# widkyyu/Goal-conditioned-Reinforcement-Learning-with-environmental-and-policy-priors

Measured on AMD Instinct MI355X. Metric: env-steps/sec, higher is better.
Workload: dtype u8

## Files before the change

### goal-conditioned-reinforcement-learning-with-environmental-and-policy-priors_amd/_lib.py

```python
import ctypes as C
import os
import subprocess

_PKG_DIR = os.path.dirname(os.path.abspath(__file__))
LIB_PATH = os.path.join(_PKG_DIR, "libtwoarmy_hip.so")
CSRC_DIR = os.path.join(_PKG_DIR, "csrc")

TW_CELLS = 289
TW_REC_WORDS = 48
TW_DRAW_WORDS = 8
TW_F_AUTORESET = 1
TW_F_POLICY_IDX = 2
TW_F_MATRIX_CODE = 4
TW_F_SLAB_HIPMALLOC = 8

FIELDS = dict(AX=0, AY=1, DIR=2, STEP_COUNT=3, STEP_MOVE=4, PONE=5, PATROL=6, UP1=7, RIGHT2=8, UPD_LONG=9,
              UPD_HORIZ=10, RISK=11, FIRST_ROOM2=12, OBX=13, OBY=16, O1X=19, O1Y=22, O1_VALID=25, O2X=26,
              O2Y=30, O2_VALID=34, GOAL_X=35, GOAL_Y=36, T=37, ERROR=38, MAX_STEPS=39, EPISODES=40,
              LAST_REWARD=41, LAST_TERM=42, LAST_TRUNC=43, WALL_I1=44, WALL_I2=45)

ENV_ERRORS = {1: AttributeError, 2: AssertionError, 3: TypeError}


class TwoarmyLibraryError(RuntimeError):
    pass


def build(force=False):
    cmd = ["make", "-s", "-C", CSRC_DIR] + (["-B"] if force else [])
    subprocess.check_call(cmd)
    return LIB_PATH


_vp = C.c_void_p


class TwOutputs(C.Structure):
    _fields_ = [("obs", _vp), ("matrix", _vp), ("pos", _vp), ("reward", _vp), ("terminated", _vp), ("truncated", _vp),
                ("obs_pitch", C.c_int), ("mat_pitch", C.c_int), ("T", C.c_int), ("n_envs", C.c_int), ("flags", C.c_int),
                ("device", C.c_int), ("backing", C.c_int), ("slab_bytes", C.c_uint64), ("slab", _vp)]


_SIGS = {
    "tw_create": (C.c_int, [C.POINTER(_vp), C.c_int, C.c_int, C.c_int, C.c_int, C.c_uint64, C.c_uint32]),
    "tw_destroy": (C.c_int, [_vp]),
    "tw_reset": (C.c_int, [_vp, _vp, _vp, C.c_int, _vp]),
    "tw_step": (C.c_int, [_vp, _vp, _vp, _vp, C.c_int, _vp, C.c_int, _vp, _vp, _vp, _vp, C.c_int, _vp]),
    "tw_rollout": (C.c_int, [_vp, C.c_int, _vp, _vp, _vp, C.c_int, _vp, C.c_int, _vp, _vp, _vp, _vp, C.c_int, _vp]),
    "tw_set_envs_per_wave": (C.c_int, [_vp, C.c_int]),
    "tw_set_pipeline": (C.c_int, [_vp, C.c_int]),
    "tw_fallback_count": (C.c_int, [_vp, C.POINTER(C.c_int)]),
    "tw_fill_actions": (C.c_int, [_vp, C.c_int, _vp, _vp]),
    "tw_state_ptrs": (C.c_int, [_vp, C.POINTER(_vp), C.POINTER(_vp), C.POINTER(_vp)]),
    "tw_get_state_host": (C.c_int, [_vp, _vp, _vp, _vp]),
    "tw_set_state_host": (C.c_int, [_vp, _vp, _vp, _vp]),
    "tw_gen_obs": (C.c_int, [_vp, C.c_int, _vp, C.c_int, _vp]),
    "tw_n_envs": (C.c_int, [_vp]),
    "tw_view_size": (C.c_int, [_vp]),
    "tw_last_hip_error": (C.c_int, []),
    "tw_version": (C.c_char_p, []),
    "tw_build_id": (C.c_char_p, []),
    "tw_last_error_message": (C.c_char_p, []),
    "tw_alloc_outputs": (C.c_int, [_vp, C.c_int, C.c_int, C.POINTER(TwOutputs)]),
    "tw_free_outputs": (C.c_int, [C.POINTER(TwOutputs)]),
    "tw_abi_sizeof_outputs": (C.c_int, []),
    "tw_time_rollout": (C.c_int, [_vp, C.c_int, _vp, _vp, C.c_int, _vp, C.c_int, _vp, _vp, _vp, _vp, C.c_int, C.c_int, _vp,
                                  C.POINTER(C.c_float)]),
}

_f, _i, _u64, _i64 = C.c_float, C.c_int, C.c_uint64, C.c_int64
_SIGS.update({
    "ppo_sample": (C.c_int, [_vp, _i, _i, _vp, _u64, _u64, _vp, _vp, _vp]),
    "ppo_sample_dev": (C.c_int, [_vp, _i, _i, _vp, _u64, _u64, _vp, _vp, _vp, _vp]),
    "ppo_gae": (C.c_int, [_vp, _vp, _vp, _vp, _f, _f, _i, _i, _i, _vp, _vp, _vp, _vp]),
    "ppo_adv_norm": (C.c_int, [_vp, _i64, _f, _vp, _vp]),
    "ppo_loss_fwd_bwd": (C.c_int, [_vp, _vp, _vp, _vp, _vp, _vp, _i, _i, _f, _f, _vp, _vp, _vp, _vp, _vp]),
    "ppo_loss_fwd_bwd_masked": (C.c_int, [_vp, _vp, _vp, _vp, _vp, _vp, _i, _i, _i, _f, _f, _vp, _vp, _vp, _vp, _vp]),
    "ppo_gather_stack": (C.c_int, [_vp, _i, _vp, _i, _vp, _vp, _vp, _vp, _vp, _i, _vp, _vp, _vp]),
    "mg_gen_obs": (C.c_int, [_vp, _vp, _vp, _i, _i, _i, _vp, _vp, _vp, _vp, _i, _i, _vp, _i, _vp, _vp]),
    "mg_step": (C.c_int, [_vp, _vp, _i, _i, _i, _vp, _vp, _vp, _vp, _vp, _i, _vp, _vp, _vp, _vp, _vp]),
    "mg_render_tile_index": (C.c_int, [_i, _i, _i, _i, _i]),
    "mg_render_atlas_bytes": (_i64, [_i]),
    "mg_render_constants": (C.c_int, [C.POINTER(C.c_double)]),
    "mg_render_build_atlas": (C.c_int, [_i, _vp, _vp]),
    "mg_render": (C.c_int, [_vp, _vp, _vp, _i, _i, _i, _vp, _vp, _vp, _i, _vp, _i, _vp, _vp, _i, _vp, _i64, _vp, _vp]),
    "mg_highlight_mask": (C.c_int, [_vp, _i, _i, _i, _vp, _vp, _vp, _i, _i, _vp, _vp]),
    "ppo_her_relabel": (C.c_int, [_vp, _vp, _vp, _vp, _vp, _vp, _u64, C.c_uint32, C.c_uint32, _i, _i, _i, _vp, _vp, _vp,
                                  _vp, _vp, _vp, _vp, _vp]),
    "ppo_her_relabel_window": (C.c_int, [_vp, _vp, _vp, _vp, _vp, _vp, _u64, C.c_uint32, C.c_uint32, _i, _i, _i, _i, _vp,
                                         _vp, _vp, _vp, _vp, _vp, _vp, _vp]),
    "ppo_lstm_cell": (C.c_int, [_vp, _vp, C.c_longlong, _vp, _vp, _vp, _i, _i, _vp]),
    "ppo_decoder_frames": (C.c_int, [_vp, _i, _vp, _vp, _vp, _vp, _vp, C.c_float, _vp, _vp]),
    "ppo_gather_stack_u8": (C.c_int, [_vp, _i, _vp, _i, _vp, _vp, _vp, _vp, _vp, _i, _vp, _vp, _vp]),
    "ppo_age_scan": (C.c_int, [_vp, _vp, _vp, _i, _i, _vp, _vp]),
    "ppo_episode_scan": (C.c_int, [_vp, _vp, _vp, _i, _i, _vp, _vp, _vp, _vp, _vp]),
    "ppo_episode_summary": (C.c_int, [_vp, _vp, _vp, _vp, _vp, _vp, _i, _i, _i, C.c_double, C.c_double, _vp, _vp, _vp, _vp,
                                      _vp, _vp]),
    "ppo_episode_summary_workspace": (C.c_int, [_i, _i]),
    "ppo_bias_relu_nhwc": (C.c_int, [_vp, _vp, _i64, _i, _vp]),
    "ppo_conv1_up4_bias_relu": (C.c_int, [_vp, _i, _i, _vp, _vp, _vp, _vp]),
    "ppo_conv1_up4_bias_relu_c": (C.c_int, [_vp, _i, _i, _i, _vp, _vp, _vp, _vp]),
    "ppo_conv1_up4_bwd_groups": (C.c_int, [_i]),
    "ppo_conv1_up4_bwd": (C.c_int, [_vp, _i, _i, _vp, _vp, _vp, _vp, _vp]),
    "ppo_relu_bwd_bias_grad_nhwc_blocks": (C.c_int, [_i64, _i]),
    "ppo_relu_bwd_bias_grad_nhwc": (C.c_int, [_vp, _vp, _vp, _vp, _i64, _i, _vp]),
})

_lib = None


def exported_symbols():
    return sorted(_SIGS)


def lib():
    global _lib
    if _lib is None:
        if not os.path.exists(LIB_PATH):
            raise TwoarmyLibraryError(
                "%s not built: run `python -c 'import __graft_entry__ as g; g.build()'` "
                "(hipcc --offload-arch=gfx950); there is no CPU fallback" % LIB_PATH)
        import torch
        try:
            h = C.CDLL(LIB_PATH)
        except OSError as ex:
            raise TwoarmyLibraryError("cannot load %s: %s" % (LIB_PATH, ex)) from ex
        for name, (res, args) in _SIGS.items():
            try:
                fn = getattr(h, name)
            except AttributeError as ex:
                raise TwoarmyLibraryError("%s lacks symbol %s" % (LIB_PATH, name)) from ex
            fn.restype, fn.argtypes = res, args
        runtimes = set()
        try:
            with open("/proc/self/maps") as f:
                for line in f:
                    if "libamdhip64" in line:
                        runtimes.add(line.split()[-1])
        except OSError:
            pass
        if h.tw_abi_sizeof_outputs() != C.sizeof(TwOutputs):
            raise TwoarmyLibraryError("struct tw_outputs: the library has %d bytes, the ctypes mirror %d"
                                      % (h.tw_abi_sizeof_outputs(), C.sizeof(TwOutputs)))
        if len(runtimes) > 1:
            raise TwoarmyLibraryError("two HIP runtimes mapped (%s): import torch before loading %s"
                                      % (sorted(runtimes), LIB_PATH))
        _lib = h
    return _lib


def check(rc, what):
    if rc != 0:
        raise TwoarmyLibraryError("%s failed: rc=%d hipError=%d %s" % (
            what, rc, lib().tw_last_hip_error(), lib().tw_last_error_message().decode()))
```

### goal-conditioned-reinforcement-learning-with-environmental-and-policy-priors_amd/csrc/ppo_kernels.hip

```cpp

#include <hip/hip_runtime.h>
#include <float.h>
#include <stdint.h>

#include "twoarmy.h"
#include "twoarmy_ppo.h"

namespace {

constexpr float CAT_EPS = FLT_EPSILON;

__device__ __forceinline__ void philox4x32_10(uint32_t k0, uint32_t k1, uint32_t &c0, uint32_t &c1, uint32_t &c2,
                                              uint32_t &c3) {
#pragma unroll
    for (int r = 0; r < 10; ++r) {
        const uint32_t lo0 = 0xD2511F53u * c0, hi0 = __umulhi(0xD2511F53u, c0);
        const uint32_t lo1 = 0xCD9E8D57u * c2, hi1 = __umulhi(0xCD9E8D57u, c2);
        const uint32_t n0 = hi1 ^ c1 ^ k0, n2 = hi0 ^ c3 ^ k1;
        c0 = n0; c1 = lo1; c2 = n2; c3 = lo0;
        k0 += 0x9E3779B9u; k1 += 0xBB67AE85u;
    }
}

template <int A>
__global__ void ppo_sample_kernel(const float *__restrict__ probs, int B, const float *__restrict__ uniforms,
                                  uint32_t k0, uint32_t k1, uint64_t offset, const uint64_t *__restrict__ offset_dev,
                                  int32_t *__restrict__ action, float *__restrict__ logp) {
    const int b = blockIdx.x * blockDim.x + threadIdx.x;
    if (b >= B) return;
    float p[A];
    float sum = 0.f;
#pragma unroll
    for (int k = 0; k < A; ++k) { p[k] = probs[(size_t)b * A + k]; sum += p[k]; }
    float u;
    if (uniforms) u = uniforms[b];
    else {
        const uint64_t ctr = (uint64_t)b + offset + (offset_dev ? *offset_dev : 0ull);
        uint32_t c0 = (uint32_t)ctr, c1 = (uint32_t)(ctr >> 32), c2 = 0, c3 = 0x54574F53u;
        philox4x32_10(k0, k1, c0, c1, c2, c3);
        u = (float)(c0 >> 8) * (1.0f / 16777216.0f);
    }
    int a = A - 1, last = A - 1;
    float cum = 0.f, qa = 0.f;
    bool found = false;
#pragma unroll
    for (int k = 0; k < A; ++k) {
        const float q = p[k] / sum;
        cum += q;
        if (q > 0.f) last = k;
        if (!found && cum > u) { a = k; found = true; }
    }
    if (!found) a = last;
#pragma unroll
    for (int k = 0; k < A; ++k) if (k == a) qa = p[k] / sum;
    action[b] = a;
    logp[b] = logf(fminf(fmaxf(qa, CAT_EPS), 1.0f - CAT_EPS));
}

__global__ __launch_bounds__(256) void ppo_bias_relu_kernel(float4 *__restrict__ y, const float4 *__restrict__ bias,
                                                            size_t n4, int c4) {
    const size_t stride = (size_t)gridDim.x * blockDim.x;
    for (size_t i = (size_t)blockIdx.x * blockDim.x + threadIdx.x; i < n4; i += stride) {
        float4 v = y[i];
        const float4 b = bias[i % c4];
        v.x = fmaxf(v.x + b.x, 0.f); v.y = fmaxf(v.y + b.y, 0.f);
        v.z = fmaxf(v.z + b.z, 0.f); v.w = fmaxf(v.w + b.w, 0.f);
        y[i] = v;
    }
}

__global__ __launch_bounds__(256) void ppo_relu_bwd_bias_grad_kernel(const float4 *__restrict__ gy,
                                                                     const float4 *__restrict__ y,
                                                                     float4 *__restrict__ gx,
                                                                     float4 *__restrict__ partial, size_t n_pixels,
                                                                     int c4, int pixels_per_block) {
    __shared__ float4 red[256];
    const int rows = 256 / c4;
    const int cq = threadIdx.x % c4, row = threadIdx.x / c4;
    const size_t p0 = (size_t)blockIdx.x * pixels_per_block;
    const size_t p1 = p0 + pixels_per_block < n_pixels ? p0 + pixels_per_block : n_pixels;
    float4 acc = make_float4(0.f, 0.f, 0.f, 0.f);
    if (row < rows) {
        for (size_t px = p0 + row; px < p1; px += rows) {
            const size_t i = px * c4 + cq;
            const float4 g = gy[i], v = y[i];
            float4 o;
            o.x = v.x > 0.f ? g.x : 0.f; o.y = v.y > 0.f ? g.y : 0.f;
            o.z = v.z > 0.f ? g.z : 0.f; o.w = v.w > 0.f ? g.w : 0.f;
            gx[i] = o;
            acc.x += o.x; acc.y += o.y; acc.z += o.z; acc.w += o.w;
        }
    }
    red[threadIdx.x] = acc;
    __syncthreads();
    if (row == 0) {
        for (int r = 1; r < rows; ++r) {
            const float4 o = red[r * c4 + cq];
            acc.x += o.x; acc.y += o.y; acc.z += o.z; acc.w += o.w;
        }
        partial[(size_t)blockIdx.x * c4 + cq] = acc;
    }
}

template <int F, int CQ>
__global__ __launch_bounds__(256) void ppo_conv1_up4_kernel(const float *__restrict__ frames, const float4 *__restrict__ wf,
                                                            const float4 *__restrict__ bias, float4 *__restrict__ out, int B) {
    __shared__ float xs[F * 18 * 18];
    constexpr int SLOTS = 256 / CQ;
    const int b = blockIdx.x, tid = threadIdx.x;
    const int cq = tid % CQ, slot = tid / CQ;
    const float *src = frames + (size_t)b * F * 289;
    for (int i = tid; i < F * 324; i += 256) {
        const int c = i / 324, r = i - c * 324, y = r / 18, x = r - y * 18;
        xs[i] = (y < 17 && x < 17) ? src[c * 289 + y * 17 + x] : 0.f;
    }
    __syncthreads();
    const float4 bv = bias[cq];
    float4 *dst = out + (size_t)b * 1089 * CQ;
#pragma unroll 1
    for (int ph = 0; ph < 4; ++ph) {
        const int py = ph >> 1, px = ph & 1;
        float4 w[4 * F];
#pragma unroll
        for (int k = 0; k < 4 * F; ++k) w[k] = wf[(ph * 4 * F + k) * CQ + cq];
        const int ny = 17 - py, nx = 17 - px;
        for (int q = slot; q < ny * nx; q += SLOTS) {
            const int m = q / nx, n = q - m * nx;
            float4 acc = bv;
#pragma unroll
            for (int t = 0; t < 4; ++t) {
                const int ty = t >> 1, tx = t & 1;
#pragma unroll
                for (int c = 0; c < F; ++c) {
                    const float xv = xs[c * 324 + (m + ty) * 18 + n + tx];
                    const float4 ww = w[t * F + c];
                    acc.x = fmaf(xv, ww.x, acc.x); acc.y = fmaf(xv, ww.y, acc.y);
                    acc.z = fmaf(xv, ww.z, acc.z); acc.w = fmaf(xv, ww.w, acc.w);
                }
            }
            acc.x = fmaxf(acc.x, 0.f); acc.y = fmaxf(acc.y, 0.f); acc.z = fmaxf(acc.z, 0.f); acc.w = fmaxf(acc.w, 0.f);
            dst[((2 * m + py) * 33 + 2 * n + px) * CQ + cq] = acc;
        }
    }
}

template <int F>
__global__ __launch_bounds__(256) void ppo_conv1_up4_bwd_kernel(const float *__restrict__ frames, const float4 *__restrict__ gy,
                                                                const float4 *__restrict__ y, float4 *__restrict__ gw_part,
                                                                float4 *__restrict__ gb_part, int B) {
    __shared__ float xs[F * 18 * 18];
    __shared__ float4 red[256];
    const int tid = threadIdx.x, cq = tid & 15, slot = tid >> 4;
    const int ph = blockIdx.y, py = ph >> 1, px = ph & 1;
    const int ny = 17 - py, nx = 17 - px;
    float4 acc[4 * F];
#pragma unroll
    for (int k = 0; k < 4 * F; ++k) acc[k] = make_float4(0.f, 0.f, 0.f, 0.f);
    float4 accb = make_float4(0.f, 0.f, 0.f, 0.f);
    for (int b = blockIdx.x; b < B; b += gridDim.x) {
        __syncthreads();
        const float *src = frames + (size_t)b * F * 289;
        for (int i = tid; i < F * 324; i += 256) {
            const int c = i / 324, r = i - c * 324, yy = r / 18, xx = r - yy * 18;
            xs[i] = (yy < 17 && xx < 17) ? src[c * 289 + yy * 17 + xx] : 0.f;
        }
        __syncthreads();
        const size_t base = (size_t)b * 1089 * 16;
        for (int q = slot; q < ny * nx; q += 16) {
            const int m = q / nx, n = q - m * nx;
            const size_t o = base + (size_t)((2 * m + py) * 33 + 2 * n + px) * 16 + cq;
            const float4 gv = gy[o], yv = y[o];
            float4 g;
            g.x = yv.x > 0.f ? gv.x : 0.f; g.y = yv.y > 0.f ? gv.y : 0.f;
            g.z = yv.z > 0.f ? gv.z : 0.f; g.w = yv.w > 0.f ? gv.w : 0.f;
            accb.x += g.x; accb.y += g.y; accb.z += g.z; accb.w += g.w;
#pragma unroll
            for (int t = 0; t < 4; ++t) {
                const int ty = t >> 1, tx = t & 1;
#pragma unroll
                for (int c = 0; c < F; ++c) {
                    const float xv = xs[c * 324 + (m + ty) * 18 + n + tx];
                    float4 &a = acc[t * F + c];
                    a.x = fmaf(xv, g.x, a.x); a.y = fmaf(xv, g.y, a.y); a.z = fmaf(xv, g.z, a.z); a.w = fmaf(xv, g.w, a.w);
                }
            }
        }
    }
    const size_t wbase = ((size_t)blockIdx.x * 4 + ph) * (4 * F) * 16;
#pragma unroll
    for (int k = 0; k <= 4 * F; ++k) {
        __syncthreads();
        red[tid] = k < 4 * F ? acc[k < 4 * F ? k : 0] : accb;
        __syncthreads();
        if (slot == 0) {
            float4 sum = red[cq];
            for (int r = 1; r < 16; ++r) {
                const float4 o = red[r * 16 + cq];
                sum.x += o.x; sum.y += o.y; sum.z += o.z; sum.w += o.w;
            }
            if (k < 4 * F) gw_part[wbase + (size_t)k * 16 + cq] = sum;
            else gb_part[((size_t)blockIdx.x * 4 + ph) * 16 + cq] = sum;
        }
    }
}

constexpr int GT = 64;

template <int GN>
__global__ __launch_bounds__(256) void ppo_gae_kernel(const float *__restrict__ reward, const float *__restrict__ value,
                                                      const float *__restrict__ next_value,
                                                      const uint8_t *__restrict__ done, float gamma, float lambda,
                                                      int use_done_mask, int T, int N, float *__restrict__ adv,
                                                      float *__restrict__ target, float *__restrict__ ret) {
    __shared__ float sd[GT][GN + 1];
    __shared__ float sc[GT][GN + 1];
    __shared__ float carry[GN];
    constexpr int ROWS = 256 / GN;
    const int tid = threadIdx.x, tx = tid % GN, ty = tid / GN;
    const int n = blockIdx.x * GN + tx;
    if (tid < GN) carry[tid] = 0.f;
    const int nchunks = (T + GT - 1) / GT;
    for (int ch = nchunks - 1; ch >= 0; --ch) {
        const int t0 = ch * GT;
        __syncthreads();
        for (int r = ty; r < GT; r += ROWS) {
            const int t = t0 + r;
            float d = 0.f, c = 1.f;
            if (t < T && n < N) {
                const size_t i = (size_t)t * N + n;
                const float cut = (use_done_mask && done[i]) ? 0.f : 1.f;
                const float tv = reward[i] + (gamma * next_value[i]) * cut;
                if (target) target[i] = tv;
                d = tv - value[i];
                c = gamma * lambda * cut;
            }
            sd[r][tx] = d; sc[r][tx] = c;
        }
        __syncthreads();
        const int wave = tid >> 6, lane = tid & 63;
        for (int e = wave * (GN / 4); e < (wave + 1) * (GN / 4); ++e) {
            float d = sd[lane][e], c = sc[lane][e];
#pragma unroll
            for (int off = 1; off < 64; off <<= 1) {
                const float d2 = __shfl_down(d, off), c2 = __shfl_down(c, off);
                if (lane + off < 64 && c != 0.f) { d = fmaf(c, d2, d); c = c * c2; }
            }
            const float a = c != 0.f ? fmaf(c, carry[e], d) : d;
            sd[lane][e] = a;
            const float a0 = __shfl(a, 0);
            if (lane == 0) carry[e] = a0;
        }
        __syncthreads();
        for (int r = ty; r < GT; r += ROWS) {
            const int t = t0 + r;
            if (t < T && n < N) {
                const size_t i = (size_t)t * N + n;
                const float a = sd[r][tx];
                if (adv) adv[i] = a;
                if (ret) ret[i] = a + value[i];
            }
        }
    }
}

__global__ __launch_bounds__(256) void ppo_moments_kernel(const float *__restrict__ x, int64_t n, double *__restrict__ ws) {
    __shared__ double s1[256], s2[256];
    double a = 0.0, b = 0.0;
    for (int64_t i = (int64_t)blockIdx.x * 256 + threadIdx.x; i < n; i += (int64_t)gridDim.x * 256) {
        const double v = (double)x[i];
        a += v; b += v * v;
    }
    s1[threadIdx.x] = a; s2[threadIdx.x] = b;
    __syncthreads();
    for (int s = 128; s > 0; s >>= 1) {
        if ((int)threadIdx.x < s) { s1[threadIdx.x] += s1[threadIdx.x + s]; s2[threadIdx.x] += s2[threadIdx.x + s]; }
        __syncthreads();
    }
    if (threadIdx.x == 0) { ws[2 * blockIdx.x] = s1[0]; ws[2 * blockIdx.x + 1] = s2[0]; }
}

__global__ __launch_bounds__(256) void ppo_normalise_kernel(float *__restrict__ x, int64_t n, float eps,
                                                            const double *__restrict__ ws, int nblocks) {
    __shared__ float s_mean, s_inv;
    __shared__ double r1[256], r2[256];
    r1[threadIdx.x] = (int)threadIdx.x < nblocks ? ws[2 * threadIdx.x] : 0.0;
// ... 722 lines not shown
    const int64_t per_block = (M + nblocks - 1) / nblocks;
    const int per_thread = (int)((per_block + 255) / 256);
    hipStream_t st = (hipStream_t)stream;
    hipLaunchKernelGGL(ppo_episode_partial_kernel, dim3(nblocks), dim3(256), 0, st, ep_return, ep_length, terminated,
                       truncated, reward, action, M, per_block, per_thread, keep, gain, workspace);
    hipLaunchKernelGGL(ppo_episode_finalize_kernel, dim3(1), dim3(64), 0, st, workspace, nblocks, A, score, summary,
                       action_hist, reward_hist);
    return check_launch();
}

int ppo_bias_relu_nhwc(float *y, const float *bias, int64_t n_pixels, int C, void *stream) {
    if (!y || !bias || n_pixels <= 0 || C <= 0 || (C & 3) || ((uintptr_t)y & 15u) || ((uintptr_t)bias & 15u)) return TW_E_ARG;
    const size_t n4 = (size_t)n_pixels * (C / 4);
    const int grid = (int)((n4 + 255) / 256 < 8192 ? (n4 + 255) / 256 : 8192);
    hipLaunchKernelGGL(ppo_bias_relu_kernel, dim3(grid), dim3(256), 0, (hipStream_t)stream, reinterpret_cast<float4 *>(y),
                       reinterpret_cast<const float4 *>(bias), n4, C / 4);
    return check_launch();
}

int ppo_relu_bwd_bias_grad_nhwc_blocks(int64_t n_pixels, int C) {
    if (n_pixels <= 0 || C <= 0 || (C & 3) || C > 256) return TW_E_ARG;
    const int64_t want = (n_pixels + 511) / 512;
    return (int)(want < 4096 ? want : 4096);
}

int ppo_relu_bwd_bias_grad_nhwc(const float *gy, const float *y, float *gx, float *partial, int64_t n_pixels, int C,
                                void *stream) {
    const int blocks = ppo_relu_bwd_bias_grad_nhwc_blocks(n_pixels, C);
    if (blocks <= 0 || !gy || !y || !gx || !partial || (((uintptr_t)gy | (uintptr_t)y | (uintptr_t)gx | (uintptr_t)partial) & 15u))
        return TW_E_ARG;
    const int ppb = (int)((n_pixels + blocks - 1) / blocks);
    hipLaunchKernelGGL(ppo_relu_bwd_bias_grad_kernel, dim3(blocks), dim3(256), 0, (hipStream_t)stream,
                       reinterpret_cast<const float4 *>(gy), reinterpret_cast<const float4 *>(y),
                       reinterpret_cast<float4 *>(gx), reinterpret_cast<float4 *>(partial), (size_t)n_pixels, C / 4, ppb);
    return check_launch();
}

int ppo_conv1_up4_bias_relu(const float *frames, int B, int F, const float *folded_w, const float *bias, float *out,
                            void *stream) {
    return ppo_conv1_up4_bias_relu_c(frames, B, F, 64, folded_w, bias, out, stream);
}

int ppo_conv1_up4_bias_relu_c(const float *frames, int B, int F, int C_out, const float *folded_w, const float *bias,
                              float *out, void *stream) {
    if (!frames || !folded_w || !bias || !out || B <= 0 || ((uintptr_t)out & 15u) || ((uintptr_t)folded_w & 15u) ||
        ((uintptr_t)bias & 15u))
        return TW_E_ARG;
    hipStream_t st = (hipStream_t)stream;
#define PPO_CONV1_LAUNCH(FF, CQQ)                                                                                        \
    hipLaunchKernelGGL((ppo_conv1_up4_kernel<FF, CQQ>), dim3(B), dim3(256), 0, st, frames,                               \
                       reinterpret_cast<const float4 *>(folded_w), reinterpret_cast<const float4 *>(bias),               \
                       reinterpret_cast<float4 *>(out), B)
    if (F == 4 && C_out == 64) PPO_CONV1_LAUNCH(4, 16);
    else if (F == 8 && C_out == 64) PPO_CONV1_LAUNCH(8, 16);
    else if (F == 1 && C_out == 16) PPO_CONV1_LAUNCH(1, 4);
    else return TW_E_ARG;
#undef PPO_CONV1_LAUNCH
    return check_launch();
}

int ppo_conv1_up4_bwd_groups(int B) { return B <= 0 ? TW_E_ARG : (B < 256 ? B : 256); }

int ppo_conv1_up4_bwd(const float *frames, int B, int F, const float *gy, const float *y, float *gw_partial,
                      float *gb_partial, void *stream) {
    const int groups = ppo_conv1_up4_bwd_groups(B);
    if (groups <= 0 || !frames || !gy || !y || !gw_partial || !gb_partial ||
        (((uintptr_t)gy | (uintptr_t)y | (uintptr_t)gw_partial | (uintptr_t)gb_partial) & 15u))
        return TW_E_ARG;
    hipStream_t st = (hipStream_t)stream;
    const dim3 grid(groups, 4), block(256);
    if (F == 4)
        hipLaunchKernelGGL(ppo_conv1_up4_bwd_kernel<4>, grid, block, 0, st, frames, reinterpret_cast<const float4 *>(gy),
                           reinterpret_cast<const float4 *>(y), reinterpret_cast<float4 *>(gw_partial),
                           reinterpret_cast<float4 *>(gb_partial), B);
    else if (F == 8)
        hipLaunchKernelGGL(ppo_conv1_up4_bwd_kernel<8>, grid, block, 0, st, frames, reinterpret_cast<const float4 *>(gy),
                           reinterpret_cast<const float4 *>(y), reinterpret_cast<float4 *>(gw_partial),
                           reinterpret_cast<float4 *>(gb_partial), B);
    else
        return TW_E_ARG;
    return check_launch();
}

int ppo_decoder_frames(const float *z, int n_frames, const float *w1, const float *b1, const float *w2, const float *b2,
                       const float *kfold, float b3, float *frames, void *stream) {
    if (!z || !w1 || !b1 || !w2 || !b2 || !kfold || !frames || n_frames <= 0) return TW_E_ARG;
    const int grid = n_frames < 512 ? n_frames : 512;
    hipLaunchKernelGGL(ppo_decoder_frames_kernel, dim3(grid), dim3(256), 0, (hipStream_t)stream, z, n_frames, w1, b1, w2,
                       b2, kfold, b3, frames);
    return check_launch();
}

int ppo_lstm_cell(const float *gates_a, const float *gates_b, long long ldb, const float *bias, float *c, float *h, int B,
                  int H, void *stream) {
    if ((!gates_a && !gates_b) || !c || !h || B <= 0 || H <= 0 || (H & 3) ||
        (((uintptr_t)gates_a | (uintptr_t)c | (uintptr_t)h) & 15u))
        return TW_E_ARG;
    if (gates_b && ((((uintptr_t)gates_b) & 15u) || (ldb & 3) || ldb < 4LL * H)) return TW_E_ARG;
    if (bias && (((uintptr_t)bias) & 15u)) return TW_E_ARG;
    const long long n = (long long)B * (H / 4);
    if (n > 0x7fffffffLL) return TW_E_ARG;
    hipLaunchKernelGGL(ppo_lstm_cell_kernel, dim3((unsigned)((n + 255) / 256)), dim3(256), 0, (hipStream_t)stream,
                       reinterpret_cast<const float4 *>(gates_a), reinterpret_cast<const float4 *>(gates_b), ldb / 4,
                       reinterpret_cast<const float4 *>(bias), reinterpret_cast<float4 *>(c), reinterpret_cast<float4 *>(h),
                       B, H / 4);
    return check_launch();
}

}
```

### goal-conditioned-reinforcement-learning-with-environmental-and-policy-priors_amd/ppo_ops.py

```python
import ctypes as C

import torch

from . import _lib


def _p(t, dtype=None):
    if t is None:
        return None
    assert t.is_cuda and t.is_contiguous(), "PPO kernels take contiguous device tensors"
    if dtype is not None:
        assert t.dtype == dtype, "expected %s got %s" % (dtype, t.dtype)
    return C.c_void_p(t.data_ptr())


def _stream(t):
    return C.c_void_p(torch.cuda.current_stream(t.device).cuda_stream)


def sample(probs, uniforms=None, seed=0, offset=0, offset_dev=None):
    B, A = probs.shape
    action = torch.empty(B, dtype=torch.int32, device=probs.device)
    logp = torch.empty(B, dtype=torch.float32, device=probs.device)
    _lib.check(_lib.lib().ppo_sample_dev(_p(probs, torch.float32), B, A, _p(uniforms, torch.float32), seed, offset,
# ... 130 lines not shown
    _lib.check(fn(*args, None, _p(counts), None, None, None, None, None, _stream(pos)), "ppo_her_relabel_window")
    incl = torch.cumsum(counts.long(), 0)
    H = int(incl[-1])
    offsets = (incl - counts.long()).contiguous()
    out = dict(t=torch.empty(H, dtype=torch.int32, device=dev), n=torch.empty(H, dtype=torch.int32, device=dev),
               goal=torch.empty((H, 2), dtype=torch.float32, device=dev),
               reward=torch.empty(H, dtype=torch.float32, device=dev), done=torch.empty(H, dtype=torch.uint8, device=dev),
               counts=counts)
    if H:
        _lib.check(fn(*args, _p(offsets), _p(counts), _p(out["t"]), _p(out["n"]), _p(out["goal"]), _p(out["reward"]),
                      _p(out["done"]), _stream(pos)), "ppo_her_relabel_window")
    return out


class _ConvBiasReLU(torch.autograd.Function):

    @staticmethod
    def forward(ctx, x, w, b, stride):
        y = torch.ops.aten.convolution(x, w, None, list(stride), [0, 0], [1, 1], False, [0, 0], 1)
        assert y.is_contiguous(memory_format=torch.channels_last), "conv epilogue kernels need channels-last activations"
        B, Cc, H, W = y.shape
        _lib.check(_lib.lib().ppo_bias_relu_nhwc(C.c_void_p(y.data_ptr()), _p(b.detach(), torch.float32), B * H * W, Cc,
                                                 _stream(y)), "ppo_bias_relu_nhwc")
        ctx.save_for_backward(x, w, y)
        ctx.stride = list(stride)
        return y

    @staticmethod
    def backward(ctx, gy):
        x, w, y = ctx.saved_tensors
        gy = gy.contiguous(memory_format=torch.channels_last)
        B, Cc, H, W = y.shape
        npix = B * H * W
        blocks = _lib.lib().ppo_relu_bwd_bias_grad_nhwc_blocks(npix, Cc)
        g = torch.empty_like(y)
        partial = torch.empty((blocks, Cc), dtype=torch.float32, device=y.device)
        _lib.check(_lib.lib().ppo_relu_bwd_bias_grad_nhwc(C.c_void_p(gy.data_ptr()), C.c_void_p(y.data_ptr()),
                                                          C.c_void_p(g.data_ptr()), _p(partial), npix, Cc, _stream(y)),
                   "ppo_relu_bwd_bias_grad_nhwc")
        gx, gw, _ = torch.ops.aten.convolution_backward(g, x, w, None, ctx.stride, [0, 0], [1, 1], False, [0, 0], 1,
                                                        [bool(ctx.needs_input_grad[0]), True, False])
        return gx, gw, partial.sum(0), None


def conv_bias_relu(x, weight, bias, stride):
    assert x.is_cuda and x.dtype == torch.float32 and x.is_contiguous(memory_format=torch.channels_last)
    return _ConvBiasReLU.apply(x, weight, bias, tuple(stride))


def fold_conv1_weights(w):
    O, F = w.shape[0], w.shape[1]
    w = w.detach().reshape(O, F, 4, 4).float()
    z = torch.zeros_like(w[:, :, 0:1, :])
    rows = torch.stack([torch.cat([w.sum(2, keepdim=True), z], 2),
                        torch.cat([w[:, :, 0:2].sum(2, keepdim=True), w[:, :, 2:4].sum(2, keepdim=True)], 2)], 0)
    zc = torch.zeros_like(rows[..., 0:1])
    cols = torch.stack([torch.cat([rows.sum(-1, keepdim=True), zc], -1),
                        torch.cat([rows[..., 0:2].sum(-1, keepdim=True), rows[..., 2:4].sum(-1, keepdim=True)], -1)], 1)
    return cols.permute(0, 1, 4, 5, 3, 2).contiguous()


@torch.no_grad()
def conv1_up4_bias_relu_infer(frames, weight, bias):
    B, F, _ = frames.shape
    Cout = weight.shape[0]
    y = torch.empty((B, Cout, 33, 33), dtype=torch.float32, device=frames.device, memory_format=torch.channels_last)
    wf = fold_conv1_weights(weight)
    _lib.check(_lib.lib().ppo_conv1_up4_bias_relu_c(_p(frames.contiguous(), torch.float32), B, F, Cout, _p(wf),
                                                    _p(bias.contiguous(), torch.float32), C.c_void_p(y.data_ptr()),
                                                    _stream(y)), "ppo_conv1_up4_bias_relu_c")
    return y


class _Conv1Up4(torch.autograd.Function):

    @staticmethod
    def forward(ctx, frames, w, b, wf):
        B, F, _ = frames.shape
        y = torch.empty((B, w.shape[0], 33, 33), dtype=torch.float32, device=frames.device,
                        memory_format=torch.channels_last)
        if wf is None:
            wf = fold_conv1_weights(w)
        fr = frames.contiguous()
        _lib.check(_lib.lib().ppo_conv1_up4_bias_relu(_p(fr, torch.float32), B, F, _p(wf), _p(b.detach().contiguous()),
                                                      C.c_void_p(y.data_ptr()), _stream(y)), "ppo_conv1_up4_bias_relu")
        ctx.save_for_backward(fr, w, y)
        return y

    @staticmethod
    def backward(ctx, gy):
        fr, w, y = ctx.saved_tensors
        gy = gy.contiguous(memory_format=torch.channels_last)
        B, F = fr.shape[0], fr.shape[1]
        groups = _lib.lib().ppo_conv1_up4_bwd_groups(B)
        gw_part = torch.empty((groups, 2, 2, 2, 2, F, 64), dtype=torch.float32, device=y.device)
        gb_part = torch.empty((groups, 4, 64), dtype=torch.float32, device=y.device)
        _lib.check(_lib.lib().ppo_conv1_up4_bwd(_p(fr, torch.float32), B, F, C.c_void_p(gy.data_ptr()), C.c_void_p(y.data_ptr()),
                                                _p(gw_part), _p(gb_part), _stream(y)), "ppo_conv1_up4_bwd")
        return None, unfold_conv1_grad(gw_part.sum(0)).to(w.dtype), gb_part.sum((0, 1)), None


def unfold_conv1_grad(gwf):
    ty = torch.tensor([[0, 0, 0, 0], [0, 0, 1, 1]], device=gwf.device)
    out = None
    for py in (0, 1):
        for px in (0, 1):
            g = gwf[py, px][ty[py]][:, ty[px]]
            out = g if out is None else out + g
    return out.permute(3, 2, 0, 1).contiguous()


def conv1_up4_bias_relu(frames, weight, bias, folded=None):
    assert frames.is_cuda and frames.dtype == torch.float32 and weight.shape[2:] == (4, 4) and weight.shape[0] == 64
    return _Conv1Up4.apply(frames, weight, bias, folded)


def fold_decoder_tail(w3):
    m = torch.tensor([[0., 0., 1., 1.], [1., 1., 1., 1.], [1., 1., 0., 0.]], dtype=w3.dtype, device=w3.device)
    return torch.einsum("ur,crs,vs->cuv", m, w3[:, 0], m).mul_(1.0 / 16.0).contiguous()


def decoder_frames(z, w1, b1, w2, b2, w3, b3):
    assert z.dim() == 4 and tuple(z.shape[1:]) == (64, 4, 4) and z.dtype == torch.float32
    z = z.contiguous()
    n = z.shape[0]
    out = torch.empty((n, 289), dtype=torch.float32, device=z.device)
    if n:
        _lib.check(_lib.lib().ppo_decoder_frames(_p(z), n, _p(w1.detach().contiguous(), torch.float32),
                                                 _p(b1.detach().contiguous(), torch.float32),
                                                 _p(w2.detach().contiguous(), torch.float32),
                                                 _p(b2.detach().contiguous(), torch.float32),
                                                 _p(fold_decoder_tail(w3.detach())), 0.0, _p(out), _stream(z)),
                   "ppo_decoder_frames")
        out += b3.detach().view(1, 1)
    return out


def lstm_cell_(gates, c, gates_b=None, bias=None):
    B, H = c.shape
    H4 = 4 * H
    assert c.dtype == torch.float32 and (gates is not None or gates_b is not None)
    assert gates is None or (gates.shape == (B, H4) and gates.dtype == torch.float32)
    pb, ldb = None, 0
    if gates_b is not None:
        assert gates_b.shape == (B, H4) and gates_b.stride(1) == 1 and gates_b.dtype == torch.float32 and gates_b.is_cuda
        pb, ldb = C.c_void_p(gates_b.data_ptr()), gates_b.stride(0) if B > 1 else H4
    h = torch.empty_like(c)
    _lib.check(_lib.lib().ppo_lstm_cell(_p(gates), pb, ldb, _p(bias), _p(c), _p(h), B, H, _stream(c)), "ppo_lstm_cell")
    return h
```

### include/twoarmy_ppo.h

```cpp
#ifndef TWOARMY_PPO_H
#define TWOARMY_PPO_H

#include <stdint.h>

#ifdef __cplusplus
extern "C" {
#endif

int ppo_sample(const float *probs, int B, int A, const float *uniforms, uint64_t seed, uint64_t offset,
               int32_t *action, float *logp, void *stream);
int ppo_sample_dev(const float *probs, int B, int A, const float *uniforms, uint64_t seed, uint64_t offset,
                   const uint64_t *offset_dev, int32_t *action, float *logp, void *stream);

int ppo_gae(const float *reward, const float *value, const float *next_value, const uint8_t *done,
            float gamma, float lambda, int use_done_mask, int T, int N, float *adv, float *target, float *ret,
            void *stream);

int ppo_adv_norm(float *adv, int64_t n, float eps, double *workspace, void *stream);

int ppo_loss_fwd_bwd(const float *probs, const int32_t *action, const float *old_logp, const float *adv,
                     const float *value, const float *target_v, int B, int A, float clip, float ent_coef,
                     float *losses, float *grad_probs, float *grad_value, float *workspace, void *stream);
int ppo_loss_fwd_bwd_masked(const float *probs, const int32_t *action, const float *old_logp, const float *adv,
                            const float *value, const float *target_v, int B, int n_valid, int A, float clip,
                            float ent_coef, float *losses, float *grad_probs, float *grad_value, float *workspace,
                            void *stream);

int ppo_gather_stack(const float *frames, int frame_pitch, const float *pos_frames, int N,
                     const int32_t *k_idx, const int32_t *n_idx, const int32_t *age, const float *init_frame,
                     const float *init_pos, int B, float *out, float *pos_out, void *stream);

int ppo_gather_stack_u8(const uint8_t *frames, int frame_pitch, const float *pos_frames, int N,
                        const int32_t *k_idx, const int32_t *n_idx, const int32_t *age, const float *init_frame,
                        const float *init_pos, int B, float *out, float *pos_out, void *stream);

int ppo_age_scan(const uint8_t *terminated, const uint8_t *truncated, const int32_t *age0, int T, int N,
                 int32_t *age, void *stream);

int ppo_episode_scan(const float *reward, const uint8_t *terminated, const uint8_t *truncated, int T, int N,
                     double *carry_return, int32_t *carry_length, double *ep_return, int32_t *ep_length, void *stream);

int ppo_episode_summary(const double *ep_return, const int32_t *ep_length, const uint8_t *terminated,
                        const uint8_t *truncated, const float *reward, const int32_t *action, int A, int T, int N,
                        double keep, double gain, double *score, double *summary, int64_t *action_hist,
                        int64_t *reward_hist, double *workspace, void *stream);
int ppo_episode_summary_workspace(int T, int N);

int ppo_her_relabel(const float *pos, const uint8_t *terminated, const uint8_t *truncated, const int32_t *age0,
                    const float *reward, const int32_t *choices, uint64_t seed, uint32_t env_id0, uint32_t step0, int T,
                    int N, int max_goals, const int64_t *offsets, int32_t *counts, int32_t *out_t, int32_t *out_n,
                    float *out_goal, float *out_reward, uint8_t *out_done, void *stream);
int ppo_her_relabel_window(const float *pos, const uint8_t *terminated, const uint8_t *truncated, const int32_t *age0,
                           const float *reward, const int32_t *choices, uint64_t seed, uint32_t env_id0, uint32_t step0,
                           int T, int N, int max_goals, int skip, const int64_t *offsets, int32_t *counts, int32_t *out_t,
                           int32_t *out_n, float *out_goal, float *out_reward, uint8_t *out_done, void *stream);

int ppo_bias_relu_nhwc(float *y, const float *bias, int64_t n_pixels, int C, void *stream);
int ppo_relu_bwd_bias_grad_nhwc_blocks(int64_t n_pixels, int C);
int ppo_relu_bwd_bias_grad_nhwc(const float *gy, const float *y, float *gx, float *partial, int64_t n_pixels, int C,
                                void *stream);

int ppo_conv1_up4_bias_relu(const float *frames, int B, int F, const float *folded_w, const float *bias, float *out,
                            void *stream);
int ppo_conv1_up4_bias_relu_c(const float *frames, int B, int F, int C_out, const float *folded_w, const float *bias,
                              float *out, void *stream);

int ppo_conv1_up4_bwd_groups(int B);
int ppo_conv1_up4_bwd(const float *frames, int B, int F, const float *gy, const float *y, float *gw_partial,
                      float *gb_partial, void *stream);

int ppo_decoder_frames(const float *z, int n_frames, const float *w1, const float *b1, const float *w2, const float *b2,
                       const float *kfold, float b3, float *frames, void *stream);

int ppo_lstm_cell(const float *gates_a, const float *gates_b, long long ldb, const float *bias, float *c, float *h, int B,
                  int H, void *stream);

#ifdef __cplusplus
}
#endif
#endif
```

Baseline: 3.138 billion.

## Recompute conv1 activation in backward and accumulate weight grads with MFMA

The conv1 backward no longer saves or reads the forward output y. It recomputes the pre-activation from the frames and folded weights to build the ReLU mask. Weight-gradient accumulation uses 16x16x4 f32 MFMA instructions, and the gradient and frame loads are double-buffered across chunks and batches. This cuts saved-activation memory and backward read traffic, at the cost of redoing the forward FMAs and adding register pressure.

```diff
diff --git a/goal-conditioned-reinforcement-learning-with-environmental-and-policy-priors_amd/_lib.py b/goal-conditioned-reinforcement-learning-with-environmental-and-policy-priors_amd/_lib.py
--- a/goal-conditioned-reinforcement-learning-with-environmental-and-policy-priors_amd/_lib.py
+++ b/goal-conditioned-reinforcement-learning-with-environmental-and-policy-priors_amd/_lib.py
@@ -102,6 +102,7 @@
     "ppo_conv1_up4_bias_relu_c": (C.c_int, [_vp, _i, _i, _i, _vp, _vp, _vp, _vp]),
     "ppo_conv1_up4_bwd_groups": (C.c_int, [_i]),
     "ppo_conv1_up4_bwd": (C.c_int, [_vp, _i, _i, _vp, _vp, _vp, _vp, _vp]),
+    "ppo_conv1_up4_bwd_recompute": (C.c_int, [_vp, _i, _i, _vp, _vp, _vp, _vp, _vp, _vp]),
     "ppo_relu_bwd_bias_grad_nhwc_blocks": (C.c_int, [_i64, _i]),
     "ppo_relu_bwd_bias_grad_nhwc": (C.c_int, [_vp, _vp, _vp, _vp, _i64, _i, _vp]),
 })
diff --git a/goal-conditioned-reinforcement-learning-with-environmental-and-policy-priors_amd/csrc/ppo_kernels.hip b/goal-conditioned-reinforcement-learning-with-environmental-and-policy-priors_amd/csrc/ppo_kernels.hip
--- a/goal-conditioned-reinforcement-learning-with-environmental-and-policy-priors_amd/csrc/ppo_kernels.hip
+++ b/goal-conditioned-reinforcement-learning-with-environmental-and-policy-priors_amd/csrc/ppo_kernels.hip
@@ -102,6 +102,23 @@
     }
 }
 
+template <int F>
+__device__ __forceinline__ float4 conv1_up4_pre(const float *xs, int m, int n, const float4 (&w)[4 * F], float4 bv) {
+    float4 acc = bv;
+#pragma unroll
+    for (int t = 0; t < 4; ++t) {
+        const int ty = t >> 1, tx = t & 1;
+#pragma unroll
+        for (int c = 0; c < F; ++c) {
+            const float xv = xs[c * 324 + (m + ty) * 18 + n + tx];
+            const float4 ww = w[t * F + c];
+            acc.x = fmaf(xv, ww.x, acc.x); acc.y = fmaf(xv, ww.y, acc.y);
+            acc.z = fmaf(xv, ww.z, acc.z); acc.w = fmaf(xv, ww.w, acc.w);
+        }
+    }
+    return acc;
+}
+
 template <int F, int CQ>
 __global__ __launch_bounds__(256) void ppo_conv1_up4_kernel(const float *__restrict__ frames, const float4 *__restrict__ wf,
                                                             const float4 *__restrict__ bias, float4 *__restrict__ out, int B) {
@@ -126,18 +143,7 @@
         const int ny = 17 - py, nx = 17 - px;
         for (int q = slot; q < ny * nx; q += SLOTS) {
             const int m = q / nx, n = q - m * nx;
-            float4 acc = bv;
-#pragma unroll
-            for (int t = 0; t < 4; ++t) {
-                const int ty = t >> 1, tx = t & 1;
-#pragma unroll
-                for (int c = 0; c < F; ++c) {
-                    const float xv = xs[c * 324 + (m + ty) * 18 + n + tx];
-                    const float4 ww = w[t * F + c];
-                    acc.x = fmaf(xv, ww.x, acc.x); acc.y = fmaf(xv, ww.y, acc.y);
-                    acc.z = fmaf(xv, ww.z, acc.z); acc.w = fmaf(xv, ww.w, acc.w);
-                }
-            }
+            float4 acc = conv1_up4_pre<F>(xs, m, n, w, bv);
             acc.x = fmaxf(acc.x, 0.f); acc.y = fmaxf(acc.y, 0.f); acc.z = fmaxf(acc.z, 0.f); acc.w = fmaxf(acc.w, 0.f);
             dst[((2 * m + py) * 33 + 2 * n + px) * CQ + cq] = acc;
         }
@@ -201,6 +207,147 @@
             if (k < 4 * F) gw_part[wbase + (size_t)k * 16 + cq] = sum;
             else gb_part[((size_t)blockIdx.x * 4 + ph) * 16 + cq] = sum;
         }
+    }
+}
+
+typedef float conv1_f32x4 __attribute__((ext_vector_type(4)));
+
+template <int F>
+__global__ __launch_bounds__(256, F == 4 ? 2 : 1) void ppo_conv1_up4_bwd_recompute_kernel(
+    const float *__restrict__ frames, const float4 *__restrict__ gy, const float4 *__restrict__ wf,
+    const float4 *__restrict__ bias, float4 *__restrict__ gw_part, float4 *__restrict__ gb_part, int B) {
+    constexpr int U = F == 4 ? 4 : 2;
+    constexpr int MT = F / 4;
+    constexpr int NF = (F * 324 + 255) / 256;
+    __shared__ float xs[F * 18 * 18];
+    __shared__ float4 red[256];
+    const int tid = threadIdx.x, cq = tid & 15, slot = tid >> 4, lane = tid & 63, wave = tid >> 6;
+    const int ph = blockIdx.y, py = ph >> 1, px = ph & 1;
+    const int ny = 17 - py, nx = 17 - px, npix = ny * nx;
+    const int nch = ((npix + 15) / 16 + U - 1) / U;
+    float4 w[4 * F];
+#pragma unroll
+    for (int k = 0; k < 4 * F; ++k) w[k] = wf[(ph * 4 * F + k) * 16 + cq];
+    const float4 bv = bias[cq];
+    int aoff[MT];
+#pragma unroll
+    for (int mt = 0; mt < MT; ++mt) {
+        const int k = mt * 16 + cq, t = k / F, c = k - t * F;
+        aoff[mt] = c * 324 + (t >> 1) * 18 + (t & 1);
+    }
+    conv1_f32x4 acc[MT][4];
+#pragma unroll
+    for (int mt = 0; mt < MT; ++mt)
+#pragma unroll
+        for (int e = 0; e < 4; ++e) acc[mt][e] = conv1_f32x4{0.f, 0.f, 0.f, 0.f};
+    float4 accb = make_float4(0.f, 0.f, 0.f, 0.f);
+
+    auto split = [&](int q, int &m, int &n) { m = px ? q >> 4 : q / 17; n = q - m * nx; };
+    auto load_frame = [&](int b, float (&fx)[NF]) {
+        const float *src = frames + (size_t)b * F * 289;
+#pragma unroll
+        for (int j = 0; j < NF; ++j) {
+            const int i = tid + 256 * j;
+            const int c = i / 324, r = i - c * 324, yy = r / 18, xx = r - yy * 18;
+            fx[j] = (i < F * 324 && yy < 17 && xx < 17) ? src[c * 289 + yy * 17 + xx] : 0.f;
+        }
+    };
+    auto load_chunk = [&](int b, int ch, float4 (&buf)[U]) {
+        const size_t base = (size_t)(b < B ? b : B - 1) * 1089 * 16;
+#pragma unroll
+        for (int j = 0; j < U; ++j) {
+            const int q = (ch * U + j) * 16 + slot;
+            int m, n;
+            split(q < npix ? q : npix - 1, m, n);
+            buf[j] = gy[base + (size_t)((2 * m + py) * 33 + 2 * n + px) * 16 + cq];
+        }
+    };
+
+    auto consume = [&](int ch, const float4 (&buf)[U]) {
+#pragma unroll
+        for (int j = 0; j < U; ++j) {
+            const int q0 = (ch * U + j) * 16;
+            if (q0 < npix) {
+                const int q = q0 + slot;
+                const bool valid = q < npix;
+                int m, n;
+                split(valid ? q : 0, m, n);
+                const float4 pre = conv1_up4_pre<F>(xs, m, n, w, bv);
+                const float4 gv = buf[j];
+                float4 g;
+                g.x = (valid && pre.x > 0.f) ? gv.x : 0.f; g.y = (valid && pre.y > 0.f) ? gv.y : 0.f;
+                g.z = (valid && pre.z > 0.f) ? gv.z : 0.f; g.w = (valid && pre.w > 0.f) ? gv.w : 0.f;
+                if (valid) { accb.x += g.x; accb.y += g.y; accb.z += g.z; accb.w += g.w; }
+#pragma unroll
+                for (int mt = 0; mt < MT; ++mt) {
+                    const float xa = valid ? xs[aoff[mt] + m * 18 + n] : 0.f;
+                    acc[mt][0] = __builtin_amdgcn_mfma_f32_16x16x4f32(xa, g.x, acc[mt][0], 0, 0, 0);
+                    acc[mt][1] = __builtin_amdgcn_mfma_f32_16x16x4f32(xa, g.y, acc[mt][1], 0, 0, 0);
+                    acc[mt][2] = __builtin_amdgcn_mfma_f32_16x16x4f32(xa, g.z, acc[mt][2], 0, 0, 0);
+                    acc[mt][3] = __builtin_amdgcn_mfma_f32_16x16x4f32(xa, g.w, acc[mt][3], 0, 0, 0);
+                }
+            }
+        }
+    };
+
+    float fx[NF];
+    float4 ga[U], gb[U];
+    int b = blockIdx.x;
+    load_frame(b, fx);
+    load_chunk(b, 0, ga);
+    for (; b < B; b += gridDim.x) {
+        __syncthreads();
+#pragma unroll
+        for (int j = 0; j < NF; ++j)
+            if (tid + 256 * j < F * 324) xs[tid + 256 * j] = fx[j];
+        __syncthreads();
+        const int bn = b + gridDim.x;
+        if (bn < B) load_frame(bn, fx);
+#pragma unroll 1
+        for (int ch = 0; ch < nch; ch += 2) {
+            if (ch + 1 < nch) {
+                load_chunk(b, ch + 1, gb);
+                consume(ch, ga);
+                if (ch + 2 < nch) load_chunk(b, ch + 2, ga);
+                else load_chunk(bn, 0, ga);
+                consume(ch + 1, gb);
+            } else {
+                load_chunk(bn, 0, gb);
+                consume(ch, ga);
+#pragma unroll
+                for (int j = 0; j < U; ++j) ga[j] = gb[j];
+            }
+        }
+    }
+    const size_t wbase = ((size_t)blockIdx.x * 4 + ph) * (4 * F) * 16;
+#pragma unroll
+    for (int mt = 0; mt < MT; ++mt) {
+#pragma unroll
+        for (int r = 0; r < 4; ++r) {
+            __syncthreads();
+            red[tid] = make_float4(acc[mt][0][r], acc[mt][1][r], acc[mt][2][r], acc[mt][3][r]);
+            __syncthreads();
+            if (wave == 0) {
+                float4 sum = red[lane];
+                for (int v = 1; v < 4; ++v) {
+                    const float4 o = red[v * 64 + lane];
+                    sum.x += o.x; sum.y += o.y; sum.z += o.z; sum.w += o.w;
+                }
+                const int k = mt * 16 + (lane >> 4) * 4 + r;
+                gw_part[wbase + (size_t)k * 16 + cq] = sum;
+            }
+        }
+    }
+    __syncthreads();
+    red[tid] = accb;
+    __syncthreads();
+    if (slot == 0) {
+        float4 sum = red[cq];
+        for (int r = 1; r < 16; ++r) {
+            const float4 o = red[r * 16 + cq];
+            sum.x += o.x; sum.y += o.y; sum.z += o.z; sum.w += o.w;
+        }
+        gb_part[((size_t)blockIdx.x * 4 + ph) * 16 + cq] = sum;
     }
 }
 
@@ -1089,6 +1236,26 @@
     return check_launch();
 }
 
+int ppo_conv1_up4_bwd_recompute(const float *frames, int B, int F, const float *gy, const float *folded_w, const float *bias,
+                                float *gw_partial, float *gb_partial, void *stream) {
+    const int groups = ppo_conv1_up4_bwd_groups(B);
+    if (groups <= 0 || !frames || !gy || !folded_w || !bias || !gw_partial || !gb_partial ||
+        (((uintptr_t)gy | (uintptr_t)folded_w | (uintptr_t)bias | (uintptr_t)gw_partial | (uintptr_t)gb_partial) & 15u))
+        return TW_E_ARG;
+    hipStream_t st = (hipStream_t)stream;
+    const dim3 grid(groups, 4), block(256);
+#define PPO_CONV1_BWD_LAUNCH(FF)                                                                                         \
+    hipLaunchKernelGGL(ppo_conv1_up4_bwd_recompute_kernel<FF>, grid, block, 0, st, frames,                               \
+                       reinterpret_cast<const float4 *>(gy), reinterpret_cast<const float4 *>(folded_w),                 \
+                       reinterpret_cast<const float4 *>(bias), reinterpret_cast<float4 *>(gw_partial),                   \
+                       reinterpret_cast<float4 *>(gb_partial), B)
+    if (F == 4) PPO_CONV1_BWD_LAUNCH(4);
+    else if (F == 8) PPO_CONV1_BWD_LAUNCH(8);
+    else return TW_E_ARG;
+#undef PPO_CONV1_BWD_LAUNCH
+    return check_launch();
+}
+
 int ppo_decoder_frames(const float *z, int n_frames, const float *w1, const float *b1, const float *w2, const float *b2,
                        const float *kfold, float b3, float *frames, void *stream) {
     if (!z || !w1 || !b1 || !w2 || !b2 || !kfold || !frames || n_frames <= 0) return TW_E_ARG;
diff --git a/goal-conditioned-reinforcement-learning-with-environmental-and-policy-priors_amd/ppo_ops.py b/goal-conditioned-reinforcement-learning-with-environmental-and-policy-priors_amd/ppo_ops.py
--- a/goal-conditioned-reinforcement-learning-with-environmental-and-policy-priors_amd/ppo_ops.py
+++ b/goal-conditioned-reinforcement-learning-with-environmental-and-policy-priors_amd/ppo_ops.py
@@ -236,21 +236,23 @@
         if wf is None:
             wf = fold_conv1_weights(w)
         fr = frames.contiguous()
-        _lib.check(_lib.lib().ppo_conv1_up4_bias_relu(_p(fr, torch.float32), B, F, _p(wf), _p(b.detach().contiguous()),
+        bb = b.detach().contiguous()
+        _lib.check(_lib.lib().ppo_conv1_up4_bias_relu(_p(fr, torch.float32), B, F, _p(wf), _p(bb),
                                                       C.c_void_p(y.data_ptr()), _stream(y)), "ppo_conv1_up4_bias_relu")
-        ctx.save_for_backward(fr, w, y)
+        ctx.save_for_backward(fr, w, wf, bb)
         return y
 
     @staticmethod
     def backward(ctx, gy):
-        fr, w, y = ctx.saved_tensors
+        fr, w, wf, bb = ctx.saved_tensors
         gy = gy.contiguous(memory_format=torch.channels_last)
         B, F = fr.shape[0], fr.shape[1]
         groups = _lib.lib().ppo_conv1_up4_bwd_groups(B)
-        gw_part = torch.empty((groups, 2, 2, 2, 2, F, 64), dtype=torch.float32, device=y.device)
-        gb_part = torch.empty((groups, 4, 64), dtype=torch.float32, device=y.device)
-        _lib.check(_lib.lib().ppo_conv1_up4_bwd(_p(fr, torch.float32), B, F, C.c_void_p(gy.data_ptr()), C.c_void_p(y.data_ptr()),
-                                                _p(gw_part), _p(gb_part), _stream(y)), "ppo_conv1_up4_bwd")
+        gw_part = torch.empty((groups, 2, 2, 2, 2, F, 64), dtype=torch.float32, device=gy.device)
+        gb_part = torch.empty((groups, 4, 64), dtype=torch.float32, device=gy.device)
+        _lib.check(_lib.lib().ppo_conv1_up4_bwd_recompute(_p(fr, torch.float32), B, F, C.c_void_p(gy.data_ptr()), _p(wf),
+                                                          _p(bb), _p(gw_part), _p(gb_part), _stream(gy)),
+                   "ppo_conv1_up4_bwd_recompute")
         return None, unfold_conv1_grad(gw_part.sum(0)).to(w.dtype), gb_part.sum((0, 1)), None
 
 
diff --git a/include/twoarmy_ppo.h b/include/twoarmy_ppo.h
--- a/include/twoarmy_ppo.h
+++ b/include/twoarmy_ppo.h
@@ -68,6 +68,8 @@
 int ppo_conv1_up4_bwd_groups(int B);
 int ppo_conv1_up4_bwd(const float *frames, int B, int F, const float *gy, const float *y, float *gw_partial,
                       float *gb_partial, void *stream);
+int ppo_conv1_up4_bwd_recompute(const float *frames, int B, int F, const float *gy, const float *folded_w, const float *bias,
+                                float *gw_partial, float *gb_partial, void *stream);
 
 int ppo_decoder_frames(const float *z, int n_frames, const float *w1, const float *b1, const float *w2, const float *b2,
                        const float *kfold, float b3, float *frames, void *stream);
```

Result: no change. 3.133 billion (median of 2 runs) (-0.2%).
